# IntuitionMachines/volta

Measured on AMD Instinct MI355X. Metric: image-text pairs/sec, ctrl_vilbert_base pretrain step, higher is better.
Workload: dtype bf16

## Files before the change

include/volta_hip.h:

```cpp
#ifndef VOLTA_HIP_H
#define VOLTA_HIP_H
#include <stddef.h>
#include <stdint.h>

#ifdef __cplusplus
extern "C" {
#endif

typedef void* vk_stream_t;

int vk_version(void);
const char* vk_device_arch(void);
const char* vk_last_error(void);

typedef struct vk_dropout {
    const uint64_t* seed;
    uint32_t site;
    uint32_t threshold;
    float scale;
} vk_dropout;

int vk_set_seed(uint64_t* seed_dev, uint64_t seed, vk_stream_t s);

int vk_cast_f32_bf16(const float* src, void* dst, int64_t n, vk_stream_t s);
// ... 187 lines not shown
    const void* src[VK_PAIR_MAX_SEGS];
    void* dst[VK_PAIR_MAX_SEGS];
    int64_t bytes[VK_PAIR_MAX_SEGS];
    int32_t side[VK_PAIR_MAX_SEGS];
    const int64_t* cap_idx;
    const int64_t* img_idx;
    int64_t n_items[2];
    int32_t nseg, npairs, c0, nc, i0, ni;
} vk_pair_gather_args;
int vk_pair_gather(const vk_pair_gather_args* a, vk_stream_t s);

int vk_select_rows(const int64_t* labels, int N, int mode, int inner, int outer, int off, int32_t* rows, int32_t* pos,
                   int32_t* count, vk_stream_t s);
int vk_gather_rows(const void* src, const int32_t* rows, const int32_t* count, void* dst, int H, int max_rows, vk_stream_t s);
int vk_scatter_rows_add(const void* src, const int32_t* rows, const int32_t* count, void* dst, int H, int max_rows, vk_stream_t s);
typedef struct vk_xent_args {
    const float* logits;
    const int64_t* labels;
    const int32_t* pos;
    const int32_t* count;
    float* lse;
    float* loss_sum;
    int32_t V, ld, max_rows;
} vk_xent_args;
int vk_xent_fwd(const vk_xent_args* a, vk_stream_t s);
int vk_xent_bwd(const vk_xent_args* a, void* dlogits, int ldd, const float* gscale, vk_stream_t s);
typedef struct vk_kl_args {
    const float* logits;
    const float* target;
    const int32_t* pos;
// ... 151 lines not shown
    VK_FN_CAST = 1, VK_FN_MEMSET, VK_FN_LOC_FWD, VK_FN_LOC_BWD, VK_FN_ADD_DROPOUT, VK_FN_COLSUM, VK_FN_SELECT,
    VK_FN_GATHER, VK_FN_SCATTER_ADD, VK_FN_LOSS_FINAL, VK_FN_POOL_FWD, VK_FN_POOL_BWD, VK_FN_MASK_PREP, VK_FN_MUL,
    VK_FN_VLBERT_PREP, VK_FN_VLBERT_MASKGRAD, VK_FN_ROWGROUP_SUM, VK_FN_RELU_BWD, VK_FN_COPY, VK_FN_SUM_SLABS, VK_FN_SUM_SLABS_BF16,
    VK_FN_SIDE_TAIL,
    VK_FN_QUANT_ROWS,
    VK_FN_CAST_FP8,
    VK_FN_VIS_LOSS_FWD,
    VK_FN_VIS_LOSS_BWD,
    VK_FN_NCE_NEG,
    VK_FN_TEXT_END_ROWS,
    VK_FN_VLBERT_OBJ_IDS,
    VK_FN_VLBERT_POSITIONS,
    VK_FN_HOLD,
    VK_FN_GATE,
    VK_FN_BUMP,
    VK_FN_GRAD_SEED
};
typedef struct vk_generic_args {
    int32_t fn;
    void* p[6];
    int64_t n[6];
    float f[2];
    vk_dropout drop;
} vk_generic_args;
typedef struct vk_op {
    int32_t kind, i0, i1, i2;
    const void* a;
    const void* b;
    const void* c;
} vk_op;
int vk_run_ops(const vk_op* ops, int n, vk_stream_t s);
// ... 148 lines not shown
```

volta_amd/_lib.py:

```python
import ctypes as C
import os

import torch

_HERE = os.path.dirname(os.path.abspath(__file__))
LIB_PATH = os.path.join(_HERE, "libvolta_hip_%s.so" % os.environ["VK_LIB"] if os.environ.get("VK_LIB") else "libvolta_hip.so")
GEMM_PERSISTENT, GEMM_ONE_TILE_PER_WG, GEMM_SOFT_START = 0x1000, 0x2000, 0x4000


class VoltaHipError(RuntimeError):
    pass


if not os.path.exists(LIB_PATH):
    raise ImportError(
        "volta_amd: %s not found. The HIP kernels are the product; there is no fallback path. "
        "Build with `make -C volta_amd/csrc` (hipcc --offload-arch=gfx950)." % LIB_PATH)

lib = C.CDLL(LIB_PATH)

c_p = C.c_void_p
i32 = C.c_int32
CHUNK_SKIP = 255

# ... 174 lines not shown


class GenericArgs(C.Structure):
    _fields_ = [("fn", i32), ("p", c_p * 6), ("n", C.c_int64 * 6), ("f", C.c_float * 2), ("drop", Dropout)]


class Op(C.Structure):
    _fields_ = [("kind", i32), ("i0", i32), ("i1", i32), ("i2", i32), ("a", c_p), ("b", c_p), ("c", c_p)]


(OP_GEMM, OP_LN_FWD, OP_LN_BWD, OP_ATTN_FWD, OP_ATTN_BWD, OP_EMBED_FWD, OP_EMBED_BWD, OP_XENT_FWD, OP_XENT_BWD,
 OP_KL_FWD, OP_KL_BWD, OP_GENERIC, OP_SIDE_BEGIN, OP_SIDE_END, OP_WAIT_SIDE, OP_JOIN, OP_LN_FINALIZE, OP_GEMM_FP8, OP_GEMM_CHAIN) = range(1, 20)
(FN_CAST, FN_MEMSET, FN_LOC_FWD, FN_LOC_BWD, FN_ADD_DROPOUT, FN_COLSUM, FN_SELECT, FN_GATHER, FN_SCATTER_ADD,
 FN_LOSS_FINAL, FN_POOL_FWD, FN_POOL_BWD, FN_MASK_PREP, FN_MUL, FN_VLBERT_PREP, FN_VLBERT_MASKGRAD, FN_ROWGROUP_SUM,
 FN_RELU_BWD, FN_COPY, FN_SUM_SLABS, FN_SUM_SLABS_BF16, FN_SIDE_TAIL, FN_QUANT_ROWS, FN_CAST_FP8, FN_VIS_LOSS_FWD, FN_VIS_LOSS_BWD,
 FN_NCE_NEG, FN_TEXT_END_ROWS, FN_VLBERT_OBJ_IDS, FN_VLBERT_POSITIONS, FN_HOLD, FN_GATE, FN_BUMP, FN_GRAD_SEED) = range(1, 35)


class AttnArgs(C.Structure):
    _fields_ = [("q", c_p * 2), ("k", c_p * 2), ("v", c_p * 2), ("ld", i32 * 2), ("L", i32 * 2), ("mask", c_p * 2),
                ("ctx", c_p * 2), ("ldo", i32 * 2), ("lse", c_p * 2), ("B", i32), ("nh", i32), ("gate", (i32 * 2) * 2),
                ("drop", (Dropout * 2) * 2), ("scale", C.c_float), ("dh", i32), ("probs", (c_p * 2) * 2)]


class AttnBwdArgs(C.Structure):
    _fields_ = [("dctx", c_p * 2), ("dq", c_p * 2), ("dk", c_p * 2), ("dv", c_p * 2), ("ldg", i32 * 2)]


NT, NN, TN = 0, 1, 2
EPI_BF16, EPI_GELU, EPI_MULR, EPI_ADDR, EPI_F32, EPI_RELU, EPI_F32_ACC = range(7)

# ... 27 lines not shown
_sig("vk_embed_sum_bwd", C.c_int, C.POINTER(EmbedBwdArgs), c_p)
_sig("vk_embed_bwd_workspace_bytes", C.c_int64, C.c_int, C.c_int, C.c_int, C.c_int, C.c_int)
_sig("vk_rows32", C.c_int, C.c_int)
_sig("vk_loc_linear_fwd", C.c_int, c_p, c_p, c_p, c_p, C.c_int, C.c_int, C.c_int, c_p)
_sig("vk_loc_linear_bwd", C.c_int, c_p, c_p, c_p, c_p, c_p, C.c_int, C.c_int, C.c_int, c_p)
_sig("vk_add_dropout", C.c_int, c_p, c_p, c_p, C.c_int, C.c_int, C.c_float, Dropout, C.c_int, c_p)
_sig("vk_colsum_bf16", C.c_int, c_p, c_p, c_p, C.c_int, C.c_int, C.c_int, c_p)
_sig("vk_vlbert_prep_fwd", C.c_int, c_p, C.c_int, c_p, c_p, c_p, c_p, C.c_int, C.c_int, C.c_int, Dropout, c_p)
_sig("vk_vlbert_maskgrad", C.c_int, c_p, C.c_int, C.c_int, c_p, c_p, c_p, C.c_int, C.c_int, Dropout, c_p)
_sig("vk_rowgroup_sum_bf16", C.c_int, c_p, c_p, C.c_int, C.c_int, C.c_int, c_p)
_sig("vk_relu_bwd_bf16", C.c_int, c_p, c_p, c_p, C.c_int64, c_p)
_sig("vk_copy_async", C.c_int, c_p, c_p, C.c_int64, c_p)
_sig("vk_select_rows", C.c_int, c_p, C.c_int, C.c_int, C.c_int, C.c_int, C.c_int, c_p, c_p, c_p, c_p)
_sig("vk_gather_rows", C.c_int, c_p, c_p, c_p, c_p, C.c_int, C.c_int, c_p)
_sig("vk_scatter_rows_add", C.c_int, c_p, c_p, c_p, c_p, C.c_int, C.c_int, c_p)
_sig("vk_xent_fwd", C.c_int, C.POINTER(XentArgs), c_p)
_sig("vk_xent_bwd", C.c_int, C.POINTER(XentArgs), c_p, C.c_int, c_p, c_p)
_sig("vk_kl_fwd", C.c_int, C.POINTER(KlArgs), c_p)
_sig("vk_kl_bwd", C.c_int, C.POINTER(KlArgs), c_p, C.c_int, c_p, c_p)
_sig("vk_loss_finalize", C.c_int, c_p, c_p, c_p, C.c_int, C.c_float, c_p, c_p)
_sig("vk_pool_mul_fwd", C.c_int, c_p, c_p, c_p, C.c_int, C.c_int, Dropout, c_p)
_sig("vk_pool_fuse_fwd", C.c_int, c_p, c_p, c_p, C.c_int, C.c_int, C.c_int, Dropout, c_p)
_sig("vk_pool_fuse_bwd", C.c_int, c_p, C.c_int, c_p, c_p, c_p, c_p, C.c_int, C.c_int, C.c_int, Dropout, c_p)
_sig("vk_text_end_rows", C.c_int, c_p, C.c_int, C.c_int, c_p, c_p, c_p)
_sig("vk_vlbert_obj_ids", C.c_int, c_p, c_p, C.c_int, C.c_int, c_p)
_sig("vk_lmdb_open", C.c_int, C.c_char_p, C.POINTER(c_p))
_sig("vk_lmdb_close", None, c_p)
_sig("vk_lmdb_entries", C.c_int64, c_p)
_sig("vk_lmdb_first", C.c_int, c_p)
_sig("vk_lmdb_next", C.c_int, c_p, C.POINTER(c_p), C.POINTER(C.c_size_t), C.POINTER(c_p), C.POINTER(C.c_size_t))
# ... 52 lines not shown
_sig("vk_run_ops", C.c_int, C.POINTER(Op), C.c_int, c_p)
_sig("vk_run_ops_timed", C.c_int, C.POINTER(Op), C.c_int, c_p, C.POINTER(C.c_float))
_sig("vk_ln_bwd_finalize", C.c_int, C.POINTER(LnBwdArgs), c_p)
_sig("vk_ln_fwd_pair", C.c_int, C.POINTER(LnArgs), C.POINTER(LnArgs), c_p)
_sig("vk_ln_bwd_pair", C.c_int, C.POINTER(LnBwdArgs), C.POINTER(LnBwdArgs), c_p)
_sig("vk_concap_batch", C.c_int, C.POINTER(ConcapArgs), c_p)
_sig("vk_side_join", C.c_int, c_p)
_sig("vk_side_join_from", C.c_int, c_p, c_p)
_sig("vk_side_enable", None, C.c_int)
_sig("vk_side_stream", c_p, c_p)

EXPORTS = ["vk_version", "vk_device_arch", "vk_last_error", "vk_set_seed", "vk_cast_f32_bf16", "vk_gemm_grouped", "vk_gemm_grouped_ex", "vk_gemm_chain", "vk_gemm_split_workspace_bytes", "vk_gemm_fp8_grouped", "vk_quant_rows_fp8", "vk_cast_bf16_fp8",
           "vk_ln_fwd", "vk_ln_fwd_pair", "vk_ln_bwd_partial_rows", "vk_ln_bwd", "vk_ln_bwd_pair", "vk_ln_bwd_finalize", "vk_gated_attn_fwd", "vk_gated_attn_bwd", "vk_gated_attn_lds_bytes",
           "vk_embed_sum_fwd", "vk_embed_sum_bwd", "vk_embed_bwd_workspace_bytes", "vk_rows32", "vk_loc_linear_fwd", "vk_loc_linear_bwd",
           "vk_add_dropout", "vk_colsum_bf16", "vk_vlbert_prep_fwd", "vk_vlbert_maskgrad", "vk_rowgroup_sum_bf16",
           "vk_relu_bwd_bf16", "vk_copy_async", "vk_select_rows", "vk_gather_rows", "vk_scatter_rows_add", "vk_xent_fwd",
           "vk_xent_bwd", "vk_kl_fwd", "vk_kl_bwd", "vk_loss_finalize", "vk_pool_mul_fwd", "vk_pool_mul_bwd",
           "vk_pool_fuse_fwd", "vk_pool_fuse_bwd", "vk_text_end_rows", "vk_vlbert_obj_ids", "vk_vlbert_positions", "vk_vis_loss_fwd", "vk_vis_loss_bwd", "vk_nce_negatives", "vk_task_loss_work_bytes", "vk_task_loss_fwd", "vk_task_loss_bwd",
           "vk_mask_prep", "vk_mul_bf16", "vk_grad_norm_workspace_floats", "vk_grad_norm_clip", "vk_grad_norm_clip_masked", "vk_grad_sqnorm_chunks", "vk_grad_norm_from_chunks", "vk_adamw_step", "vk_adamw_step_on", "vk_adamw_step_list", "vk_grad_sqnorm_list", "vk_grad_sqnorm_list_work_floats", "vk_grad_seed", "vk_pair_gather", "vk_radam_step", "vk_radam_step_list",
           "vk_axpy_f32", "vk_sum_slabs_f32", "vk_sum_slabs_bf16", "vk_memset_async", "vk_hold_cus", "vk_gate_wait", "vk_bump_u64", "vk_store_u64", "vk_gate_value", "vk_comm_standin", "vk_gemm_reserve_cus", "vk_side_tail", "vk_run_ops", "vk_run_ops_timed", "vk_side_join", "vk_side_join_from", "vk_side_stream", "vk_side_enable", "vk_concap_batch",
           "vk_lmdb_open", "vk_lmdb_close", "vk_lmdb_entries", "vk_lmdb_first", "vk_lmdb_next", "vk_lmdb_get", "vk_concap_record_decode", "vk_concap_records_decode", "vk_b64_decode",
           "vk_wordpiece_open", "vk_wordpiece_close", "vk_wordpiece_vocab_size", "vk_wordpiece_token_id", "vk_wordpiece_encode", "vk_wordpiece_encode_batch",
           "vk_task_batch", "vk_task_images_stage", "vk_retrieval_ranks", "vk_image_means", "vk_knn_pool_work_bytes", "vk_knn_pool"]


def check(rc):
    if rc != 0:
        raise VoltaHipError(lib.vk_last_error().decode())


def stream_ptr():
# ... 6 lines not shown
```

volta_amd/csrc/executor.cpp:

```cpp
#include "util.h"
#include <vector>
#include "../../include/volta_hip.h"

static int run_one(const vk_op& o, int i, vk_stream_t s);

#include <cstdlib>
#include <mutex>
#include <unordered_map>
namespace {
constexpr int N_SIDE_EVENTS = 16;
struct Side {
    hipStream_t stream = nullptr;
    hipEvent_t fork = nullptr, join = nullptr;
    hipEvent_t done[N_SIDE_EVENTS] = {};
    bool recorded[N_SIDE_EVENTS] = {};
    bool ok = false;
};
std::mutex g_side_mutex;
std::unordered_map<void*, Side*> g_sides;
int g_side_enabled = 1;

Side* side_lookup(vk_stream_t caller) {
    std::lock_guard<std::mutex> lock(g_side_mutex);
    auto it = g_sides.find((void*)caller);
// ... 127 lines not shown
            case VK_OP_XENT_BWD: rc = vk_xent_bwd((const vk_xent_args*)o.a, (void*)o.b, o.i0, (const float*)o.c, s); break;
            case VK_OP_KL_FWD: rc = vk_kl_fwd((const vk_kl_args*)o.a, s); break;
            case VK_OP_KL_BWD: rc = vk_kl_bwd((const vk_kl_args*)o.a, (void*)o.b, o.i0, (const float*)o.c, s); break;
            case VK_OP_GENERIC: {
                const vk_generic_args* g = (const vk_generic_args*)o.a;
                switch (g->fn) {
                    case VK_FN_CAST: rc = vk_cast_f32_bf16((const float*)g->p[0], g->p[1], g->n[0], s); break;
                    case VK_FN_MEMSET: rc = vk_memset_async(g->p[0], (int)g->n[1], g->n[0], s); break;
                    case VK_FN_LOC_FWD: rc = vk_loc_linear_fwd((const float*)g->p[0], (const float*)g->p[1], (const float*)g->p[2], g->p[3], (int)g->n[0], (int)g->n[1], (int)g->n[2], s); break;
                    case VK_FN_LOC_BWD: rc = vk_loc_linear_bwd(g->p[0], (const float*)g->p[1], (float*)g->p[2], (float*)g->p[3], (float*)g->p[4], (int)g->n[0], (int)g->n[1], (int)g->n[2], s); break;
                    case VK_FN_ADD_DROPOUT: rc = vk_add_dropout(g->p[0], g->p[1], g->p[2], (int)g->n[0], (int)g->n[1], g->f[0], g->drop, (int)g->n[2], s); break;
                    case VK_FN_COLSUM: rc = vk_colsum_bf16(g->p[0], (float*)g->p[1], (float*)g->p[2], (int)g->n[0], (int)g->n[1], (int)g->n[2], s); break;
                    case VK_FN_SELECT: rc = vk_select_rows((const int64_t*)g->p[0], (int)g->n[0], (int)g->n[1], (int)g->n[2], (int)g->n[3], (int)g->n[4], (int32_t*)g->p[1], (int32_t*)g->p[2], (int32_t*)g->p[3], s); break;
                    case VK_FN_GATHER: rc = vk_gather_rows(g->p[0], (const int32_t*)g->p[1], (const int32_t*)g->p[2], g->p[3], (int)g->n[0], (int)g->n[1], s); break;
                    case VK_FN_SCATTER_ADD: rc = vk_scatter_rows_add(g->p[0], (const int32_t*)g->p[1], (const int32_t*)g->p[2], g->p[3], (int)g->n[0], (int)g->n[1], s); break;
                    case VK_FN_LOSS_FINAL: rc = vk_loss_finalize((const float*)g->p[0], (const int32_t*)g->p[1], (const int32_t*)g->p[2], (int)g->n[0], g->f[0], (float*)g->p[3], s); break;
                    case VK_FN_POOL_FWD: rc = vk_pool_fuse_fwd(g->p[0], g->p[1], g->p[2], (int)g->n[0], (int)g->n[1], (int)g->n[3], g->drop, s); break;
                    case VK_FN_POOL_BWD: rc = vk_pool_fuse_bwd(g->p[0], (int)g->n[2], g->p[1], g->p[2], g->p[3], g->p[4], (int)g->n[0], (int)g->n[1], (int)g->n[3], g->drop, s); break;
                    case VK_FN_VIS_LOSS_FWD: rc = vk_vis_loss_fwd((const vk_vis_loss_args*)g->p[0], s); break;
                    case VK_FN_VIS_LOSS_BWD: rc = vk_vis_loss_bwd((const vk_vis_loss_args*)g->p[0], g->p[1], (int)g->n[0], (const float*)g->p[2], s); break;
                    case VK_FN_NCE_NEG: rc = vk_nce_negatives(g->drop, (int)g->n[0], (int)g->n[1], (int32_t*)g->p[0], s); break;
                    case VK_FN_TEXT_END_ROWS: rc = vk_text_end_rows((const int64_t*)g->p[0], (int)g->n[0], (int)g->n[1], (int32_t*)g->p[1], (int32_t*)g->p[2], s); break;
                    case VK_FN_VLBERT_OBJ_IDS: rc = vk_vlbert_obj_ids((const int32_t*)g->p[0], (int64_t*)g->p[1], (int)g->n[0], (int)g->n[1], s); break;
                    case VK_FN_VLBERT_POSITIONS: rc = vk_vlbert_positions((const int64_t*)g->p[0], (int)g->n[0], (int)g->n[1], (int)g->n[2], (int64_t*)g->p[1], (int64_t*)g->p[2], s); break;
                    case VK_FN_HOLD: rc = vk_hold_cus((int)g->n[0], (int)g->n[1], (int)g->n[2], s); break;
                    case VK_FN_GATE: rc = vk_gate_wait((const uint64_t*)g->p[0], (const uint64_t*)g->p[1], (int)g->n[0], (int32_t*)g->p[2], s); break;
                    case VK_FN_BUMP: rc = vk_bump_u64((uint64_t*)g->p[0], s); break;
                    case VK_FN_GRAD_SEED: rc = vk_grad_seed((const vk_grad_seed_args*)g->p[0], s); break;
                    case VK_FN_MASK_PREP: rc = vk_mask_prep((const int64_t*)g->p[0], (float*)g->p[1], (int)g->n[0], s); break;
                    case VK_FN_MUL: rc = vk_mul_bf16(g->p[0], g->p[1], g->p[2], g->n[0], (const int32_t*)g->p[3], (int)g->n[1], s); break;
// ... 20 lines not shown
```

volta_amd/csrc/heads.hip:

```cpp
#include "common.h"
#include "../../include/volta_hip.h"
#include "util.h"

namespace vk {

__global__ __launch_bounds__(1024) void select_rows_kernel(const int64_t* labels, int N, int mode, int inner, int outer, int off,
                                                           int32_t* rows, int32_t* pos, int32_t* count) {
    __shared__ int wave_tot[16];
    __shared__ int base_s;
    const int tid = threadIdx.x, lane = tid & 63, wave = tid >> 6;
    if (tid == 0) base_s = 0;
    __syncthreads();
    for (int start = 0; start < N; start += 1024) {
        const int i = start + tid;
        bool f = false;
        if (i < N) { const int64_t l = labels[i]; f = mode ? (l == 1) : (l != -1); }
        const unsigned long long bal = __ballot(f);
        const int before = __popcll(bal & ((1ull << lane) - 1ull));
        if (lane == 0) wave_tot[wave] = __popcll(bal);
        __syncthreads();
        int wbase = base_s;
        for (int w = 0; w < wave; ++w) wbase += wave_tot[w];
        if (f) {
            const int j = wbase + before;
// ... 15 lines not shown
    for (int c = lane * 8; c < H; c += 512) *(u32x4*)(dst + (size_t)i * H + c) = *(const u32x4*)(src + r * H + c);
}

__global__ __launch_bounds__(256) void scatter_rows_add_kernel(const uint16_t* src, const int32_t* rows, const int32_t* count, uint16_t* dst, int H, int maxrows) {
    const int lane = threadIdx.x & 63, i = blockIdx.x * 4 + (threadIdx.x >> 6);
    const int n = min(*count, maxrows);
    if (i >= n) return;
    const size_t r = (size_t)rows[i];
    for (int c = lane * 4; c < H; c += 256) {
        const u32x2 a = *(const u32x2*)(src + (size_t)i * H + c), b = *(const u32x2*)(dst + r * H + c);
        *(u32x2*)(dst + r * H + c) = u32x2{pack2bf(bf2f(a[0] & 0xFFFF) + bf2f(b[0] & 0xFFFF), bf2f(a[0] >> 16) + bf2f(b[0] >> 16)),
                                           pack2bf(bf2f(a[1] & 0xFFFF) + bf2f(b[1] & 0xFFFF), bf2f(a[1] >> 16) + bf2f(b[1] >> 16))};
    }
}

__device__ __forceinline__ float block_max(float v, float* sh) {
    v = wave_max(v);
    const int lane = threadIdx.x & 63, wave = threadIdx.x >> 6;
    __syncthreads();
    if (lane == 0) sh[wave] = v;
    __syncthreads();
    float r = sh[0];
    for (int w = 1; w < (int)(blockDim.x >> 6); ++w) r = fmaxf(r, sh[w]);
    return r;
}
__device__ __forceinline__ float block_sum(float v, float* sh) {
    v = wave_sum(v);
    const int lane = threadIdx.x & 63, wave = threadIdx.x >> 6;
    __syncthreads();
    if (lane == 0) sh[wave] = v;
// ... 148 lines not shown
    hipLaunchKernelGGL(select_rows_kernel, dim3(1), dim3(1024), 0, (hipStream_t)s, labels, N, mode, inner, outer, off, rows, pos, count);
    return check_launch("vk_select_rows");
}
extern "C" int vk_gather_rows(const void* src, const int32_t* rows, const int32_t* count, void* dst, int H, int max_rows, vk_stream_t s) {
    if (H % 8) return set_error("vk_gather_rows: H %% 8 != 0");
    if (max_rows <= 0) return 0;
    hipLaunchKernelGGL(gather_rows_kernel, dim3((max_rows + 3) / 4), dim3(256), 0, (hipStream_t)s, (const uint16_t*)src, rows, count, (uint16_t*)dst, H, max_rows);
    return check_launch("vk_gather_rows");
}
extern "C" int vk_scatter_rows_add(const void* src, const int32_t* rows, const int32_t* count, void* dst, int H, int max_rows, vk_stream_t s) {
    if (H % 4) return set_error("vk_scatter_rows_add: H %% 4 != 0");
    if (max_rows <= 0) return 0;
    hipLaunchKernelGGL(scatter_rows_add_kernel, dim3((max_rows + 3) / 4), dim3(256), 0, (hipStream_t)s, (const uint16_t*)src, rows, count, (uint16_t*)dst, H, max_rows);
    return check_launch("vk_scatter_rows_add");
}
extern "C" int vk_xent_fwd(const vk_xent_args* a, vk_stream_t s) {
    if (a->max_rows <= 0) return 0;
    hipLaunchKernelGGL(xent_fwd_kernel, dim3(a->max_rows), dim3(256), 0, (hipStream_t)s, *a);
    return check_launch("vk_xent_fwd");
}
extern "C" int vk_xent_bwd(const vk_xent_args* a, void* dlogits, int ldd, const float* gscale, vk_stream_t s) {
    if (a->max_rows <= 0) return 0;
    if (ldd < a->V) return set_error("vk_xent_bwd: ldd < V");
    hipLaunchKernelGGL(xent_bwd_kernel, dim3(a->max_rows), dim3(256), 0, (hipStream_t)s, *a, (uint16_t*)dlogits, ldd, gscale);
    return check_launch("vk_xent_bwd");
}
extern "C" int vk_kl_fwd(const vk_kl_args* a, vk_stream_t s) {
    if (a->max_rows <= 0) return 0;
    hipLaunchKernelGGL(kl_fwd_kernel, dim3(a->max_rows), dim3(256), 0, (hipStream_t)s, *a);
    return check_launch("vk_kl_fwd");
// ... 26 lines not shown
```

volta_amd/engine.py:

```python
import ctypes as C
import math
import os

import torch

from . import _lib as L
from ._lib import check, ptr
from .modules import sublayer_schedule

CHUNK = 1024
VIS_TARGET_WIDTH = {"0": 1601, "1": 2048, "2": 2048, "3": 1600, "4": 400, "5": 2048, "6": 1601}
NO_DECAY = ("bias", "LayerNorm.bias", "LayerNorm.weight")


def _round_up(x, m):
    return (x + m - 1) // m * m


class ParamArena:

    def __init__(self, model, device, prefix=""):
        named = [(prefix + n, p) for n, p in model.named_parameters()]
        byname = dict(named)
        slots, seen = [], set()
# ... 514 lines not shown
            self.taps["t%d" % n], self.taps["v%d" % n] = self.x[0], self.x[1]
        self.fwd_heads_start = len(self.fwd.ops)
        head_bwd = self._heads() if self.heads == "pretrain" else self._heads_tasks()
        self.bwd.ops = list(self.bwd_pro) + list(head_bwd)
        self.bwd_marks = [len(self.bwd.ops)]
        for ops in reversed(bwd_stages):
            self.bwd.ops += ops
            self.bwd_marks.append(len(self.bwd.ops))
        self.bwd.ops.append((L.OP_JOIN, 0, 0, 0, None, None, None))
        prefixes = [["bert.t_pooler.", "bert.v_pooler.", "cls.", "clfs_dict."]] + [pf for pf in reversed(self.stage_prefix)]
        self.param_ready_stage = {}
        for name in self.arena.params:
            self.param_ready_stage[name] = max(i for i, pf in enumerate(prefixes) if any(name.startswith(q) for q in pf))
        self.fwd.freeze()
        self.bwd.freeze()

    def _build_score(self):
        cfg, B, T, Rv = self.cfg, self.B, self.T, self.Rv
        f = self.fwd.ops
        text_subs, vision_subs, per_modality = self.split
        kinds = dict(sublayer_schedule(cfg))
        self.x, self.x8, self.level, self.bwd_pro = [None, None], [None, None], [0, 0], []
        self.masks = [self.buf("mask_t", (B, T), torch.float32), self.buf("mask_v", (B, Rv), torch.float32)]
        kind = cfg.image_embeddings

        def mask_prep(m, src=None):
            g = self.generic(L.FN_MASK_PREP, p=(src, self.masks[m]), n=(B * self.st[m].L,))
            if src is None:
                self.patch(("attention_mask", "image_attention_mask")[m], g, "p", 0)
            f.append((L.OP_GENERIC, 0, 0, 0, g, None, None))
# ... 783 lines not shown
        if has_itm and ((fm != "text" and P != cfg.v_pooler_size) or P % 64):
            raise NotImplementedError("pooler sizes must match and be multiples of 64")
        if fm == "vl-bert_vqa":
            self.unused_params |= {"bert.t_pooler.dense.weight", "bert.t_pooler.dense.bias"}
        V, Vp = cfg.vocab_size, _round_up(cfg.vocab_size, 64)
        targets = [(ix, float(w)) for ix, w in cfg.visual_target_weights.items() if w > 0]
        if not targets:
            raise NotImplementedError("no visual target with a positive weight")
        if {ix for ix, _ in targets} & {"1", "2", "5"} and cfg.add_global_imgfeat is not None:
            raise NotImplementedError("the feature-regression targets compare [B, R, 2048] predictions with the [B, R+1, 2048] input "
                                      "when a global feature is added (losses.py:28,41,108 fail on the shapes)")
        x_t, x_v = self.x
        self.sums = self.buf("loss_sums", (4,), torch.float32)
        self.losses = self.buf("losses", (3,), torch.float32)
        self.gout = self.buf("gout", (3,), torch.float32)
        f.append((L.OP_GENERIC, 0, 0, 0, self.generic(L.FN_MEMSET, p=(self.sums,), n=(16, 0)), None, None))
        pt = pv = None
        if has_itm:
            pt = self.buf("pooled_t", (B, P))
            pools = [self.prob(x_t, self.W("bert.t_pooler.dense.weight"), pt, B, P, H, T * H, H, P, bias=self.Pm("bert.t_pooler.dense.bias"))]
            if fm != "text":
                pv = self.buf("pooled_v", (B, P))
                pools.append(self.prob(x_v, self.W("bert.v_pooler.dense.weight"), pv, B, P, Hv, Rv * Hv, Hv, P, bias=self.Pm("bert.v_pooler.dense.bias")))
            self.gemm(f, L.NT, L.EPI_RELU, pools)
        elif fm == "vl-bert_vqa":
            pt = self._vqa_text_pooler(f, x_t)[0]
        n_t, n_v = self.buf("n_t", (1,), torch.int32), self.buf("n_v", (1,), torch.int32)
        rows_t, pos_t = self.buf("rows_t", (st_t.M,), torch.int32), self.buf("pos_t", (st_t.M,), torch.int32)
        g = self.generic(L.FN_SELECT, p=(None, rows_t, pos_t, n_t), n=(st_t.M, 0, T, T, 0))
        self.patch("masked_lm_labels", g, "p", 0)
# ... 68 lines not shown
                f.append((L.OP_GENERIC, 0, 0, 0, self.generic(L.FN_VIS_LOSS_FWD, p=(la,)), None, None))
            vis.append((ix, Cn, Cp, la, tag))
        f.append((L.OP_SIDE_END, 11, 0, 0, None, None, None))
        fuse = {"mul": L.FUSE_MUL, "sum": L.FUSE_SUM, "text": L.FUSE_TEXT}.get(fm)
        pdrop = self.drop(0.1)
        if has_itm:
            pooled = self.buf("pooled", (B, P))
            f.append((L.OP_GENERIC, 0, 0, 0, self.generic(L.FN_POOL_FWD, p=(pt, pv, pooled), n=(B, P, 0, fuse), drop=pdrop), None, None))
            itm = self.buf("itm_logits", (B, 64), torch.float32)
            self.gemm(f, L.NT, L.EPI_F32, [self.prob(pooled, self.W("cls.bi_seq_relationship.weight"), itm, B, 2, P, P, P, 64, bias=self.Pm("cls.bi_seq_relationship.bias"), n_store=64)])
            lse_i = self.buf("itm_lse", (B,), torch.float32)
            xi = self.k(L.XentArgs(_addr(itm), None, None, None, _addr(lse_i), _addr(self.sums[2:3]), 2, 64, B))
            self.patch("next_sentence_label", xi, "labels")
            f.append((L.OP_XENT_FWD, 0, 0, 0, xi, None, None))
        f.append((L.OP_WAIT_SIDE, 11, 0, 0, None, None, None))
        f.append((L.OP_GENERIC, 0, 0, 0, self.generic(L.FN_LOSS_FINAL, p=(self.sums, n_t, n_v, self.losses), n=(B,), f=(1.0,)), None, None))
        self.taps.update(seq_t=x_t, seq_v=x_v, pooled_t=pt, pooled_v=pv)

        b, wg = [], []
        dxh = [self._dx(m, self.level[m] % 2) for m in range(2)]
        for m in range(2):
            b.append((L.OP_GENERIC, 0, 0, 0, self.generic(L.FN_MEMSET, p=(dxh[m],), n=(dxh[m].numel() * 2, 0)), None, None))
        b.append((L.OP_SIDE_BEGIN, 0, 0, 0, None, None, None))
        dhn_v = self.tmp("head_v_d1", (Mr, Hv))
        for j, (ix, Cn, Cp, la, tag) in enumerate(vis):
            dlog_v = self.buf(tag + "_dlogits", (Mr, Cp))
            if ix == "0":
                b.append((L.OP_KL_BWD, Cp, 0, 0, la, dlog_v, self.gout[1:2]))
            else:
                b.append((L.OP_GENERIC, 0, 0, 0, self.generic(L.FN_VIS_LOSS_BWD, p=(la, dlog_v, self.gout[1:2]), n=(Cp,)), None, None))
            wdec = ci + "decoder_dict.%s." % ix
            if j == 0:
                self.gemm(b, L.NN, L.EPI_BF16, [self.prob(dlog_v, self.W(wdec + "weight"), dhn_v, Mr, Hv, Cn, Cp, Hv, Hv, dyn=n_v)])
            else:
                self.gemm(b, L.NN, L.EPI_ADDR, [self.prob(dlog_v, self.W(wdec + "weight"), dhn_v, Mr, Hv, Cn, Cp, Hv, Hv, dyn=n_v, R=dhn_v, ldr=Hv)])
            self.gemm(b, L.TN, L.EPI_F32, [self.prob(dlog_v, hn_v, self.G(wdec + "weight"), Cn, Hv, Mr, Cp, Hv, Hv, bias_grad=self.G(wdec + "bias"), dyn=n_v)])
        if cfg.image_head_ln:
            dhv = self.tmp("head_v_d2", (Mr, Hv))
            b.append((L.OP_LN_BWD, 0, 0, 0, self.ln_bwd_args(dhn_v, hv, im_mean, im_rstd, ci + "transform.LayerNorm.weight", ci + "transform.LayerNorm.bias", dhv, None, Mr, nodrop, dyn=n_v, own_partial=True, H=Hv), None, None))
        else:
            dhv = dhn_v
        du_v = self.tmp("head_v_d3", (Mr, Hv))
        b.append((L.OP_GENERIC, 0, 0, 0, self.generic(L.FN_MUL, p=(dhv, gpv, du_v, n_v), n=(Mr * Hv, Hv)), None, None))
        dhx_v = self.tmp("head_v_d2" if not cfg.image_head_ln else "head_v_d1", (Mr, Hv))
        self.gemm(b, L.NN, L.EPI_BF16, [self.prob(du_v, self.W(ci + "transform.dense.weight"), dhx_v, Mr, Hv, Hv, Hv, Hv, Hv, dyn=n_v)])
        self.gemm(b, L.TN, L.EPI_F32, [self.prob(du_v, hx_v, self.G(ci + "transform.dense.weight"), Hv, Hv, Mr, Hv, Hv, Hv, bias_grad=self.G(ci + "transform.dense.bias"), dyn=n_v)])
        b.append((L.OP_GENERIC, 0, 0, 0, self.generic(L.FN_SCATTER_ADD, p=(dhx_v, rows_v, n_v, dxh[1]), n=(Hv, Mr)), None, None))
        b.append((L.OP_SIDE_END, 13, 0, 0, None, None, None))
        dlog_t = self.buf("lm_dlogits", (st_t.M, Vp))
        b.append((L.OP_XENT_BWD, Vp, 0, 0, xa, dlog_t, self.gout[0:1]))
        dhn_t = self.tmp("head_d1", (st_t.M, H))
        nsplit = max(1, min(16, V // 1920))
        if nsplit == 1:
            self.gemm(b, L.NN, L.EPI_BF16, [self.prob(dlog_t, self.W(wword), dhn_t, st_t.M, H, V, Vp, H, H, dyn=n_t)])
        else:
            kc = _round_up(-(-V // nsplit), 64)
            stride = st_t.M * H
            slabs = self.buf("lm_dgrad_slabs", (nsplit * stride,), torch.float32)
            probs, k0, wv = [], 0, self.W(wword)
            while k0 < V:
                kk = min(kc, V - k0)
                i = len(probs)
                probs.append(self.prob(dlog_t[:, k0:], wv[k0:], slabs[i * stride:], st_t.M, H, kk, Vp, H, H, dyn=n_t))
                k0 += kc
            self.gemm(b, L.NN, L.EPI_F32, probs)
            b.append((L.OP_GENERIC, 0, 0, 0, self.generic(L.FN_SUM_SLABS_BF16, p=(dhn_t, slabs, n_t), n=(stride, len(probs), stride, H)), None, None))
        self.gemm(wg, L.TN, L.EPI_F32, [self.prob(dlog_t, hn_t, self.G(wword), V, H, st_t.M, Vp, H, H, bias_grad=self.G(c + "bias"), dyn=n_t)])
        dht = self.tmp("head_d2", (st_t.M, H))
        b.append((L.OP_LN_BWD, 0, 0, 0, self.ln_bwd_args(dhn_t, ht, lm_mean, lm_rstd, c + "transform.LayerNorm.weight", c + "transform.LayerNorm.bias", dht, None, st_t.M, nodrop, dyn=n_t), None, None))
        du_t = self.tmp("head_d3", (st_t.M, H))
        b.append((L.OP_GENERIC, 0, 0, 0, self.generic(L.FN_MUL, p=(dht, gpt, du_t, n_t), n=(st_t.M * H, H)), None, None))
        dhx_t = self.tmp("head_d1", (st_t.M, H))
        self.gemm(b, L.NN, L.EPI_BF16, [self.prob(du_t, self.W(c + "transform.dense.weight"), dhx_t, st_t.M, H, H, H, H, H, dyn=n_t)])
        self.gemm(wg, L.TN, L.EPI_F32, [self.prob(du_t, hx_t, self.G(c + "transform.dense.weight"), H, H, st_t.M, H, H, H, bias_grad=self.G(c + "transform.dense.bias"), dyn=n_t)])
        b.append((L.OP_GENERIC, 0, 0, 0, self.generic(L.FN_SCATTER_ADD, p=(dhx_t, rows_t, n_t, dxh[0]), n=(H, st_t.M)), None, None))
        poolers = []
        if has_itm:
            dlog_i = self.buf("itm_dlogits", (B, 64))
            b.append((L.OP_XENT_BWD, 64, 0, 0, xi, dlog_i, self.gout[2:3]))
            dpooled = self.buf("d_pooled", (B, P))
            wi = "cls.bi_seq_relationship."
            self.gemm(b, L.NN, L.EPI_BF16, [self.prob(dlog_i, self.W(wi + "weight"), dpooled, B, P, 2, 64, P, P)])
            self.gemm(wg, L.TN, L.EPI_F32, [self.prob(dlog_i, pooled, self.G(wi + "weight"), 2, P, B, 64, P, P, bias_grad=self.G(wi + "bias"))])
            dyt = self.buf("d_pool_t", (B, P))
            dyv = self.buf("d_pool_v", (B, P)) if pv is not None else None
            b.append((L.OP_GENERIC, 0, 0, 0, self.generic(L.FN_POOL_BWD, p=(dpooled, pt, pv, dyt, dyv), n=(B, P, P, fuse), drop=pdrop), None, None))
            poolers = [(0, dyt, x_t, T, "bert.t_pooler.dense.")] + ([(1, dyv, x_v, Rv, "bert.v_pooler.dense.")] if pv is not None else [])
        for m, dy_, xm, Lm, pre in poolers:
            Hm = self.st[m].H
            self.gemm(b, L.NN, L.EPI_ADDR, [self.prob(dy_, self.W(pre + "weight"), dxh[m], B, Hm, P, P, Hm, Lm * Hm, R=dxh[m], ldr=Lm * Hm)])
            self.gemm(wg, L.TN, L.EPI_F32, [self.prob(dy_, xm, self.G(pre + "weight"), P, Hm, B, P, Lm * Hm, Hm, bias_grad=self.G(pre + "bias"))])
        b.append((L.OP_SIDE_BEGIN, 0, 0, 0, None, None, None))
        b += wg
        b.append((L.OP_SIDE_END, 12, 0, 0, None, None, None))
        b.append((L.OP_WAIT_SIDE, 13, 0, 0, None, None, None))
        self._head_wgrad_event = 12
        return b

    def _vqa_text_pooler(self, f, x_t):
        cfg, B, H, T = self.cfg, self.B, self.H, self.T
        P = cfg.pooler_size
        if P % 64:
            raise NotImplementedError("pooler size must be a multiple of 64")
        rows, cnt = self.buf("vqa_rows", (B,), torch.int32), self.buf("vqa_cnt", (1,), torch.int32)
        g = self.generic(L.FN_TEXT_END_ROWS, p=(None, rows, cnt), n=(B, T))
        self.patch("input_ids", g, "p", 0)
        f.append((L.OP_GENERIC, 0, 0, 0, g, None, None))
        xg = self.buf("vqa_x", (B, H))
        f.append((L.OP_GENERIC, 0, 0, 0, self.generic(L.FN_GATHER, p=(x_t, rows, cnt, xg), n=(H, B)), None, None))
        pt = self.buf("pooled_t", (B, P))
# ... 232 lines not shown
```

volta_amd/modeling.py:

```python
import logging
import os

import torch
from torch import nn

from . import modules as M
from .config import BertConfig

logger = logging.getLogger(__name__)


class ArenaParameters:

    __slots__ = ("vk_model", "started", "_it")

    def __init__(self, model, it):
        self.vk_model, self.started, self._it = model, False, it

    def __iter__(self):
        return self

    def __next__(self):
        self.started = True
        return next(self._it)
# ... 232 lines not shown
        return t, B, T, Rv

    def _engine_forward(self, tensors, task_id=None, attn_maps=False):
        B, T = tensors["input_ids"].shape
        Rv = tensors["image_feat"].shape[1]
        eng = self._engine(B, T, Rv, self.training, task_id, bool(attn_maps))
        eng.arena.refresh_shadow()
        if eng.fp8:
            eng.arena.sync_optimizer()
            eng.arena.refresh_fp8()
        eng.bind_inputs(tensors)
        if self._seed_base is None:
            self._seed_base = int(torch.initial_seed())
        eng.prepare_step(self._seed_base + self._step)
        self._step += 1
        eng.run_forward()
        self._last = (eng, tensors)
        return eng.losses

    def _run_step(self, node, eager, *args):
        self.materialize()
        anchor = next((p for p in self.parameters() if p.requires_grad), None) if node is not None and torch.is_grad_enabled() else None
        if anchor is not None:
            return node.apply(self, anchor, *args)
        with torch.no_grad():
            return eager(*args)

    def _backward_begin(self, eng, absent=()):
        arena = eng.arena
        from .optimization import flush_clip
# ... 207 lines not shown

    def __init__(self, config):
        super().__init__(config)
        self.bert = BertModel(config)
        self.cls = BertPreTrainingHeads(config, self.bert.embeddings.word_embeddings.weight)
        self.visual_target_weights = config.visual_target_weights
        logger.info("model's visual targets are %s", [ix for ix, w in config.visual_target_weights.items() if w > 0])
        self.tie_weights()
        self._init_root_state()

    def tie_weights(self):
        self._tie_or_clone_weights(self.cls.predictions.decoder, self.bert.embeddings.word_embeddings)

    def _losses(self, tensors):
        losses = self._engine_forward(tensors)
        return losses[0:1].clone(), losses[1:2].clone(), losses[2:3].clone()

    def _engine_backward(self, g_lm, g_img, g_nsp):
        eng, tensors = self._last
        state = self._backward_begin(eng)
        torch.cat([g_lm.reshape(1), g_img.reshape(1), g_nsp.reshape(1)], out=eng.gout)
        self._backward_run(eng, state)

    def forward(self, input_ids, image_feat, image_loc, token_type_ids=None, attention_mask=None,
                image_attention_mask=None, masked_lm_labels=None, image_label=None, image_cls=None, obj_labels=None,
                obj_confs=None, attr_labels=None, attr_confs=None, image_attrs=None, next_sentence_label=None,
                output_all_attention_masks=False):
        if masked_lm_labels is None and next_sentence_label is None:
            return self._scores(input_ids, image_feat, image_loc, token_type_ids, attention_mask, image_attention_mask, image_label,
                                output_all_attention_masks)
        if masked_lm_labels is None or image_label is None:
            raise NotImplementedError("the pre-training step needs masked_lm_labels and image_label")
        tensors, B, T, Rv = self._prep_inputs(input_ids, image_feat, image_loc, token_type_ids, attention_mask,
                                              image_attention_mask, masked_lm_labels, image_label, image_cls, next_sentence_label,
                                              obj_labels, obj_confs, attr_labels, attr_confs)
        return self._run_step(_PretrainStep, self._losses, tensors)
# ... 242 lines not shown
```

Before: 15020.

## Replace grad memset+scatter-add with scatter-define; bind loss grads directly

Drops the memset of the head input-gradient buffers and uses a new scatter-define kernel, which writes every row: it copies the gathered gradient rows and writes zeros elsewhere. This removes a full memset pass and the read-modify-write of scatter-add. To keep ordering correct, the visual pooler backward now waits on the side stream before adding into that buffer. The change also removes several small host-side ops: the loss-output clones (the forward now gets a fresh loss buffer each step instead) and the torch.cat of upstream grads, by patching the grad pointers straight into the backward ops.

```diff
diff --git a/include/volta_hip.h b/include/volta_hip.h
--- a/include/volta_hip.h
+++ b/include/volta_hip.h
@@ -225,6 +225,7 @@
                    int32_t* count, vk_stream_t s);
 int vk_gather_rows(const void* src, const int32_t* rows, const int32_t* count, void* dst, int H, int max_rows, vk_stream_t s);
 int vk_scatter_rows_add(const void* src, const int32_t* rows, const int32_t* count, void* dst, int H, int max_rows, vk_stream_t s);
+int vk_scatter_rows_define(const void* src, const int32_t* rows, const int32_t* count, void* dst, int H, int max_rows, int M, vk_stream_t s);
 typedef struct vk_xent_args {
     const float* logits;
     const int64_t* labels;
@@ -406,7 +407,8 @@
     VK_FN_HOLD,
     VK_FN_GATE,
     VK_FN_BUMP,
-    VK_FN_GRAD_SEED
+    VK_FN_GRAD_SEED,
+    VK_FN_SCATTER_DEFINE
 };
 typedef struct vk_generic_args {
     int32_t fn;
diff --git a/volta_amd/_lib.py b/volta_amd/_lib.py
--- a/volta_amd/_lib.py
+++ b/volta_amd/_lib.py
@@ -212,7 +212,7 @@
 (FN_CAST, FN_MEMSET, FN_LOC_FWD, FN_LOC_BWD, FN_ADD_DROPOUT, FN_COLSUM, FN_SELECT, FN_GATHER, FN_SCATTER_ADD,
  FN_LOSS_FINAL, FN_POOL_FWD, FN_POOL_BWD, FN_MASK_PREP, FN_MUL, FN_VLBERT_PREP, FN_VLBERT_MASKGRAD, FN_ROWGROUP_SUM,
  FN_RELU_BWD, FN_COPY, FN_SUM_SLABS, FN_SUM_SLABS_BF16, FN_SIDE_TAIL, FN_QUANT_ROWS, FN_CAST_FP8, FN_VIS_LOSS_FWD, FN_VIS_LOSS_BWD,
- FN_NCE_NEG, FN_TEXT_END_ROWS, FN_VLBERT_OBJ_IDS, FN_VLBERT_POSITIONS, FN_HOLD, FN_GATE, FN_BUMP, FN_GRAD_SEED) = range(1, 35)
+ FN_NCE_NEG, FN_TEXT_END_ROWS, FN_VLBERT_OBJ_IDS, FN_VLBERT_POSITIONS, FN_HOLD, FN_GATE, FN_BUMP, FN_GRAD_SEED, FN_SCATTER_DEFINE) = range(1, 36)
 
 
 class AttnArgs(C.Structure):
@@ -270,6 +270,7 @@
 _sig("vk_select_rows", C.c_int, c_p, C.c_int, C.c_int, C.c_int, C.c_int, C.c_int, c_p, c_p, c_p, c_p)
 _sig("vk_gather_rows", C.c_int, c_p, c_p, c_p, c_p, C.c_int, C.c_int, c_p)
 _sig("vk_scatter_rows_add", C.c_int, c_p, c_p, c_p, c_p, C.c_int, C.c_int, c_p)
+_sig("vk_scatter_rows_define", C.c_int, c_p, c_p, c_p, c_p, C.c_int, C.c_int, C.c_int, c_p)
 _sig("vk_xent_fwd", C.c_int, C.POINTER(XentArgs), c_p)
 _sig("vk_xent_bwd", C.c_int, C.POINTER(XentArgs), c_p, C.c_int, c_p, c_p)
 _sig("vk_kl_fwd", C.c_int, C.POINTER(KlArgs), c_p)
@@ -352,7 +353,7 @@
            "vk_ln_fwd", "vk_ln_fwd_pair", "vk_ln_bwd_partial_rows", "vk_ln_bwd", "vk_ln_bwd_pair", "vk_ln_bwd_finalize", "vk_gated_attn_fwd", "vk_gated_attn_bwd", "vk_gated_attn_lds_bytes",
            "vk_embed_sum_fwd", "vk_embed_sum_bwd", "vk_embed_bwd_workspace_bytes", "vk_rows32", "vk_loc_linear_fwd", "vk_loc_linear_bwd",
            "vk_add_dropout", "vk_colsum_bf16", "vk_vlbert_prep_fwd", "vk_vlbert_maskgrad", "vk_rowgroup_sum_bf16",
-           "vk_relu_bwd_bf16", "vk_copy_async", "vk_select_rows", "vk_gather_rows", "vk_scatter_rows_add", "vk_xent_fwd",
+           "vk_relu_bwd_bf16", "vk_copy_async", "vk_select_rows", "vk_gather_rows", "vk_scatter_rows_add", "vk_scatter_rows_define", "vk_xent_fwd",
            "vk_xent_bwd", "vk_kl_fwd", "vk_kl_bwd", "vk_loss_finalize", "vk_pool_mul_fwd", "vk_pool_mul_bwd",
            "vk_pool_fuse_fwd", "vk_pool_fuse_bwd", "vk_text_end_rows", "vk_vlbert_obj_ids", "vk_vlbert_positions", "vk_vis_loss_fwd", "vk_vis_loss_bwd", "vk_nce_negatives", "vk_task_loss_work_bytes", "vk_task_loss_fwd", "vk_task_loss_bwd",
            "vk_mask_prep", "vk_mul_bf16", "vk_grad_norm_workspace_floats", "vk_grad_norm_clip", "vk_grad_norm_clip_masked", "vk_grad_sqnorm_chunks", "vk_grad_norm_from_chunks", "vk_adamw_step", "vk_adamw_step_on", "vk_adamw_step_list", "vk_grad_sqnorm_list", "vk_grad_sqnorm_list_work_floats", "vk_grad_seed", "vk_pair_gather", "vk_radam_step", "vk_radam_step_list",
diff --git a/volta_amd/csrc/executor.cpp b/volta_amd/csrc/executor.cpp
--- a/volta_amd/csrc/executor.cpp
+++ b/volta_amd/csrc/executor.cpp
@@ -165,6 +165,7 @@
                     case VK_FN_SELECT: rc = vk_select_rows((const int64_t*)g->p[0], (int)g->n[0], (int)g->n[1], (int)g->n[2], (int)g->n[3], (int)g->n[4], (int32_t*)g->p[1], (int32_t*)g->p[2], (int32_t*)g->p[3], s); break;
                     case VK_FN_GATHER: rc = vk_gather_rows(g->p[0], (const int32_t*)g->p[1], (const int32_t*)g->p[2], g->p[3], (int)g->n[0], (int)g->n[1], s); break;
                     case VK_FN_SCATTER_ADD: rc = vk_scatter_rows_add(g->p[0], (const int32_t*)g->p[1], (const int32_t*)g->p[2], g->p[3], (int)g->n[0], (int)g->n[1], s); break;
+                    case VK_FN_SCATTER_DEFINE: rc = vk_scatter_rows_define(g->p[0], (const int32_t*)g->p[1], (const int32_t*)g->p[2], g->p[3], (int)g->n[0], (int)g->n[1], (int)g->n[2], s); break;
                     case VK_FN_LOSS_FINAL: rc = vk_loss_finalize((const float*)g->p[0], (const int32_t*)g->p[1], (const int32_t*)g->p[2], (int)g->n[0], g->f[0], (float*)g->p[3], s); break;
                     case VK_FN_POOL_FWD: rc = vk_pool_fuse_fwd(g->p[0], g->p[1], g->p[2], (int)g->n[0], (int)g->n[1], (int)g->n[3], g->drop, s); break;
                     case VK_FN_POOL_BWD: rc = vk_pool_fuse_bwd(g->p[0], (int)g->n[2], g->p[1], g->p[2], g->p[3], g->p[4], (int)g->n[0], (int)g->n[1], (int)g->n[3], g->drop, s); break;
diff --git a/volta_amd/csrc/heads.hip b/volta_amd/csrc/heads.hip
--- a/volta_amd/csrc/heads.hip
+++ b/volta_amd/csrc/heads.hip
@@ -53,6 +53,26 @@
     }
 }
 
+__global__ __launch_bounds__(256) void scatter_rows_define_kernel(const uint16_t* src, const int32_t* rows, const int32_t* count, uint16_t* dst, int H, int maxrows, int M) {
+    const int lane = threadIdx.x & 63, r = blockIdx.x * 4 + (threadIdx.x >> 6);
+    if (r >= M) return;
+    const int n = min(*count, maxrows);
+    int lo = 0, hi = n;
+    while (lo < hi) {
+        const int mid = (lo + hi) >> 1;
+        if (rows[mid] < r) lo = mid + 1; else hi = mid;
+    }
+    const bool hit = lo < n && rows[lo] == r;
+    for (int c = lane * 4; c < H; c += 256) {
+        u32x2 o = u32x2{0u, 0u};
+        if (hit) {
+            const u32x2 a = *(const u32x2*)(src + (size_t)lo * H + c);
+            o = u32x2{pack2bf(bf2f(a[0] & 0xFFFF) + 0.f, bf2f(a[0] >> 16) + 0.f), pack2bf(bf2f(a[1] & 0xFFFF) + 0.f, bf2f(a[1] >> 16) + 0.f)};
+        }
+        *(u32x2*)(dst + (size_t)r * H + c) = o;
+    }
+}
+
 __device__ __forceinline__ float block_max(float v, float* sh) {
     v = wave_max(v);
     const int lane = threadIdx.x & 63, wave = threadIdx.x >> 6;
@@ -231,6 +251,13 @@
     hipLaunchKernelGGL(scatter_rows_add_kernel, dim3((max_rows + 3) / 4), dim3(256), 0, (hipStream_t)s, (const uint16_t*)src, rows, count, (uint16_t*)dst, H, max_rows);
     return check_launch("vk_scatter_rows_add");
 }
+extern "C" int vk_scatter_rows_define(const void* src, const int32_t* rows, const int32_t* count, void* dst, int H, int max_rows, int M, vk_stream_t s) {
+    if (H % 4) return set_error("vk_scatter_rows_define: H %% 4 != 0");
+    if (max_rows < 0 || M < 0) return set_error("vk_scatter_rows_define: bad arguments");
+    if (M == 0) return 0;
+    hipLaunchKernelGGL(scatter_rows_define_kernel, dim3((M + 3) / 4), dim3(256), 0, (hipStream_t)s, (const uint16_t*)src, rows, count, (uint16_t*)dst, H, max_rows, M);
+    return check_launch("vk_scatter_rows_define");
+}
 extern "C" int vk_xent_fwd(const vk_xent_args* a, vk_stream_t s) {
     if (a->max_rows <= 0) return 0;
     hipLaunchKernelGGL(xent_fwd_kernel, dim3(a->max_rows), dim3(256), 0, (hipStream_t)s, *a);
diff --git a/volta_amd/engine.py b/volta_amd/engine.py
--- a/volta_amd/engine.py
+++ b/volta_amd/engine.py
@@ -552,6 +552,22 @@
             self.param_ready_stage[name] = max(i for i, pf in enumerate(prefixes) if any(name.startswith(q) for q in pf))
         self.fwd.freeze()
         self.bwd.freeze()
+        if self.heads == "pretrain":
+            where = {id(op): i for i, op in enumerate(self.bwd.ops)}
+            self._gout_sites = [(where.get(id(site), site), k) for site, k in self._gout_sites]
+
+    def fresh_losses(self):
+        self.losses = torch.empty(3, dtype=torch.float32, device=self.dev)
+        self._loss_final.p[3] = self.losses.data_ptr()
+        return self.losses
+
+    def bind_loss_grads(self, grads=None):
+        for site, k in self._gout_sites:
+            addr = self.gout.data_ptr() + 4 * k if grads is None else grads[k].data_ptr()
+            if isinstance(site, int):
+                self.bwd.c_ops[site].c = addr
+            else:
+                site.p[2] = addr
 
     def _build_score(self):
         cfg, B, T, Rv = self.cfg, self.B, self.T, self.Rv
@@ -1365,6 +1381,7 @@
         self.sums = self.buf("loss_sums", (4,), torch.float32)
         self.losses = self.buf("losses", (3,), torch.float32)
         self.gout = self.buf("gout", (3,), torch.float32)
+        self._gout_sites = []
         f.append((L.OP_GENERIC, 0, 0, 0, self.generic(L.FN_MEMSET, p=(self.sums,), n=(16, 0)), None, None))
         pt = pv = None
         if has_itm:
@@ -1463,21 +1480,22 @@
             self.patch("next_sentence_label", xi, "labels")
             f.append((L.OP_XENT_FWD, 0, 0, 0, xi, None, None))
         f.append((L.OP_WAIT_SIDE, 11, 0, 0, None, None, None))
-        f.append((L.OP_GENERIC, 0, 0, 0, self.generic(L.FN_LOSS_FINAL, p=(self.sums, n_t, n_v, self.losses), n=(B,), f=(1.0,)), None, None))
+        self._loss_final = self.generic(L.FN_LOSS_FINAL, p=(self.sums, n_t, n_v, self.losses), n=(B,), f=(1.0,))
+        f.append((L.OP_GENERIC, 0, 0, 0, self._loss_final, None, None))
         self.taps.update(seq_t=x_t, seq_v=x_v, pooled_t=pt, pooled_v=pv)
 
         b, wg = [], []
         dxh = [self._dx(m, self.level[m] % 2) for m in range(2)]
-        for m in range(2):
-            b.append((L.OP_GENERIC, 0, 0, 0, self.generic(L.FN_MEMSET, p=(dxh[m],), n=(dxh[m].numel() * 2, 0)), None, None))
         b.append((L.OP_SIDE_BEGIN, 0, 0, 0, None, None, None))
         dhn_v = self.tmp("head_v_d1", (Mr, Hv))
         for j, (ix, Cn, Cp, la, tag) in enumerate(vis):
             dlog_v = self.buf(tag + "_dlogits", (Mr, Cp))
             if ix == "0":
                 b.append((L.OP_KL_BWD, Cp, 0, 0, la, dlog_v, self.gout[1:2]))
+                self._gout_sites.append((b[-1], 1))
             else:
                 b.append((L.OP_GENERIC, 0, 0, 0, self.generic(L.FN_VIS_LOSS_BWD, p=(la, dlog_v, self.gout[1:2]), n=(Cp,)), None, None))
+                self._gout_sites.append((b[-1][4], 1))
             wdec = ci + "decoder_dict.%s." % ix
             if j == 0:
                 self.gemm(b, L.NN, L.EPI_BF16, [self.prob(dlog_v, self.W(wdec + "weight"), dhn_v, Mr, Hv, Cn, Cp, Hv, Hv, dyn=n_v)])
@@ -1494,10 +1512,11 @@
         dhx_v = self.tmp("head_v_d2" if not cfg.image_head_ln else "head_v_d1", (Mr, Hv))
         self.gemm(b, L.NN, L.EPI_BF16, [self.prob(du_v, self.W(ci + "transform.dense.weight"), dhx_v, Mr, Hv, Hv, Hv, Hv, Hv, dyn=n_v)])
         self.gemm(b, L.TN, L.EPI_F32, [self.prob(du_v, hx_v, self.G(ci + "transform.dense.weight"), Hv, Hv, Mr, Hv, Hv, Hv, bias_grad=self.G(ci + "transform.dense.bias"), dyn=n_v)])
-        b.append((L.OP_GENERIC, 0, 0, 0, self.generic(L.FN_SCATTER_ADD, p=(dhx_v, rows_v, n_v, dxh[1]), n=(Hv, Mr)), None, None))
+        b.append((L.OP_GENERIC, 0, 0, 0, self.generic(L.FN_SCATTER_DEFINE, p=(dhx_v, rows_v, n_v, dxh[1]), n=(Hv, Mr, st_v.M)), None, None))
         b.append((L.OP_SIDE_END, 13, 0, 0, None, None, None))
         dlog_t = self.buf("lm_dlogits", (st_t.M, Vp))
         b.append((L.OP_XENT_BWD, Vp, 0, 0, xa, dlog_t, self.gout[0:1]))
+        self._gout_sites.append((b[-1], 0))
         dhn_t = self.tmp("head_d1", (st_t.M, H))
         nsplit = max(1, min(16, V // 1920))
         if nsplit == 1:
@@ -1522,11 +1541,12 @@
         dhx_t = self.tmp("head_d1", (st_t.M, H))
         self.gemm(b, L.NN, L.EPI_BF16, [self.prob(du_t, self.W(c + "transform.dense.weight"), dhx_t, st_t.M, H, H, H, H, H, dyn=n_t)])
         self.gemm(wg, L.TN, L.EPI_F32, [self.prob(du_t, hx_t, self.G(c + "transform.dense.weight"), H, H, st_t.M, H, H, H, bias_grad=self.G(c + "transform.dense.bias"), dyn=n_t)])
-        b.append((L.OP_GENERIC, 0, 0, 0, self.generic(L.FN_SCATTER_ADD, p=(dhx_t, rows_t, n_t, dxh[0]), n=(H, st_t.M)), None, None))
+        b.append((L.OP_GENERIC, 0, 0, 0, self.generic(L.FN_SCATTER_DEFINE, p=(dhx_t, rows_t, n_t, dxh[0]), n=(H, st_t.M, st_t.M)), None, None))
         poolers = []
         if has_itm:
             dlog_i = self.buf("itm_dlogits", (B, 64))
             b.append((L.OP_XENT_BWD, 64, 0, 0, xi, dlog_i, self.gout[2:3]))
+            self._gout_sites.append((b[-1], 2))
             dpooled = self.buf("d_pooled", (B, P))
             wi = "cls.bi_seq_relationship."
             self.gemm(b, L.NN, L.EPI_BF16, [self.prob(dlog_i, self.W(wi + "weight"), dpooled, B, P, 2, 64, P, P)])
@@ -1535,14 +1555,19 @@
             dyv = self.buf("d_pool_v", (B, P)) if pv is not None else None
             b.append((L.OP_GENERIC, 0, 0, 0, self.generic(L.FN_POOL_BWD, p=(dpooled, pt, pv, dyt, dyv), n=(B, P, P, fuse), drop=pdrop), None, None))
             poolers = [(0, dyt, x_t, T, "bert.t_pooler.dense.")] + ([(1, dyv, x_v, Rv, "bert.v_pooler.dense.")] if pv is not None else [])
+        waited_v = False
         for m, dy_, xm, Lm, pre in poolers:
             Hm = self.st[m].H
+            if m == 1:
+                b.append((L.OP_WAIT_SIDE, 13, 0, 0, None, None, None))
+                waited_v = True
             self.gemm(b, L.NN, L.EPI_ADDR, [self.prob(dy_, self.W(pre + "weight"), dxh[m], B, Hm, P, P, Hm, Lm * Hm, R=dxh[m], ldr=Lm * Hm)])
             self.gemm(wg, L.TN, L.EPI_F32, [self.prob(dy_, xm, self.G(pre + "weight"), P, Hm, B, P, Lm * Hm, Hm, bias_grad=self.G(pre + "bias"))])
         b.append((L.OP_SIDE_BEGIN, 0, 0, 0, None, None, None))
         b += wg
         b.append((L.OP_SIDE_END, 12, 0, 0, None, None, None))
-        b.append((L.OP_WAIT_SIDE, 13, 0, 0, None, None, None))
+        if not waited_v:
+            b.append((L.OP_WAIT_SIDE, 13, 0, 0, None, None, None))
         self._head_wgrad_event = 12
         return b
 
diff --git a/volta_amd/modeling.py b/volta_amd/modeling.py
--- a/volta_amd/modeling.py
+++ b/volta_amd/modeling.py
@@ -270,6 +270,8 @@
             self._seed_base = int(torch.initial_seed())
         eng.prepare_step(self._seed_base + self._step)
         self._step += 1
+        if eng.losses is not None:
+            eng.fresh_losses()
         eng.run_forward()
         self._last = (eng, tensors)
         return eng.losses
@@ -507,12 +509,19 @@
 
     def _losses(self, tensors):
         losses = self._engine_forward(tensors)
-        return losses[0:1].clone(), losses[1:2].clone(), losses[2:3].clone()
+        return losses[0:1].detach(), losses[1:2].detach(), losses[2:3].detach()
 
     def _engine_backward(self, g_lm, g_img, g_nsp):
         eng, tensors = self._last
         state = self._backward_begin(eng)
-        torch.cat([g_lm.reshape(1), g_img.reshape(1), g_nsp.reshape(1)], out=eng.gout)
+        grads = (g_lm, g_img, g_nsp)
+        eng.gout_direct = all(g.is_cuda and g.device == eng.gout.device and g.dtype == torch.float32 and g.numel() == 1
+                              and all(st in (0, 1) for st in g.stride()) for g in grads)
+        if eng.gout_direct:
+            eng.bind_loss_grads(grads)
+        else:
+            eng.bind_loss_grads(None)
+            torch.cat([g.reshape(1) for g in grads], out=eng.gout)
         self._backward_run(eng, state)
 
     def forward(self, input_ids, image_feat, image_loc, token_type_ids=None, attention_mask=None,
```

Result: no change. 15020 (-0.0%).
